# ApsaraDB/galaxysql

Hardware: NVIDIA H100
Metric: joined+aggregated rows/sec; achieved HBM GB/s vs peak, at 1/2/4/8 H100 (higher is better)
Workload: dtype int64

## Files before the change

### galaxysql_b200/csrc/common.cuh

```cuda
#pragma once

#include <cuda_runtime.h>
#include <stdint.h>
#include <stdio.h>
#include <string.h>

#include <string>
#include <vector>

#include "../../include/gsql_gpu.h"

struct ProfEntry {
    std::string name;
    int64_t launches = 0;
    double ms = 0;
    std::vector<std::pair<cudaEvent_t, cudaEvent_t>> pending;
};

struct gsql_ctx {
    int device = 0;
    cudaStream_t stream = nullptr;
    bool own_stream = false;
    cudaStream_t copy_in = nullptr;
    cudaStream_t copy_out = nullptr;
// ... 174 lines not shown
    if (utype == GSQL_T_FP64) return gsql_hash_i64(gsql_double_bits(__longlong_as_double(k.i)));
    return gsql_hash_i64(k.i);
}
__device__ __forceinline__ int32_t gsql_row_hash(const KeySet &ks, int64_t r) {
    uint32_t h = 0;
#pragma unroll 1
    for (int c = 0; c < ks.n; c++) {
        KeyVal k = gsql_load_key(ks.c[c], r, ks.utype[c]);
        h = h * 31u + (uint32_t)gsql_key_hash(k, ks.utype[c]);
    }
    return (int32_t)h;
}

__host__ __device__ __forceinline__ uint64_t gsql_fmix64(uint64_t x) {
    x ^= x >> 33;
    x *= 0xff51afd7ed558ccdULL;
    x ^= x >> 33;
    x *= 0xc4ceb9fe1a85ec53ULL;
    x ^= x >> 33;
    return x;
}

__device__ __forceinline__ int4 ld_stream_16(const void *p) { return __ldcs(reinterpret_cast<const int4 *>(p)); }
__device__ __forceinline__ long long ld_stream_8(const void *p) { return __ldcs(reinterpret_cast<const long long *>(p)); }
__device__ __forceinline__ int ld_stream_4(const void *p) { return __ldcs(reinterpret_cast<const int *>(p)); }
__device__ __forceinline__ void st_stream_16(void *p, const int4 &v) { __stcs(reinterpret_cast<int4 *>(p), v); }
__device__ __forceinline__ void st_stream_8(void *p, long long v) { __stcs(reinterpret_cast<long long *>(p), v); }
__device__ __forceinline__ void st_stream_4(void *p, int v) { __stcs(reinterpret_cast<int *>(p), v); }

__device__ __forceinline__ uint64_t l2_policy_evict_last() {
    uint64_t pol;
    asm volatile("createpolicy.fractional.L2::evict_last.b64 %0, 1.0;" : "=l"(pol));
    return pol;
}
__device__ __forceinline__ int4 ld_keep_16(const void *p, uint64_t pol) {
    int4 v;
    asm volatile("ld.global.nc.L2::cache_hint.v4.s32 {%0,%1,%2,%3}, [%4], %5;"
                 : "=r"(v.x), "=r"(v.y), "=r"(v.z), "=r"(v.w)
                 : "l"(p), "l"(pol));
    return v;
}
__device__ __forceinline__ int4 ld_keep_16_na(const void *p, uint64_t pol) {
    int4 v;
    asm volatile("ld.global.nc.L1::no_allocate.L2::cache_hint.v4.s32 {%0,%1,%2,%3}, [%4], %5;"
                 : "=r"(v.x), "=r"(v.y), "=r"(v.z), "=r"(v.w)
                 : "l"(p), "l"(pol));
    return v;
}
__device__ __forceinline__ unsigned long long ld_keep_8(const void *p, uint64_t pol) {
    unsigned long long v;
    asm volatile("ld.global.nc.L2::cache_hint.u64 %0, [%1], %2;" : "=l"(v) : "l"(p), "l"(pol));
    return v;
}

__device__ __forceinline__ void red_add_f64_keep(double *p, double v, uint64_t pol) {
    asm volatile("red.global.add.L2::cache_hint.f64 [%0], %1, %2;" ::"l"(p), "d"(v), "l"(pol) : "memory");
}
__device__ __forceinline__ void red_add_u64_keep(unsigned long long *p, unsigned long long v, uint64_t pol) {
    asm volatile("red.global.add.L2::cache_hint.u64 [%0], %1, %2;" ::"l"(p), "l"(v), "l"(pol) : "memory");
}
__device__ __forceinline__ unsigned int ld_keep_u8(const uint8_t *p, uint64_t pol) {
    unsigned int v;
    asm volatile("ld.global.L2::cache_hint.u8 %0, [%1], %2;" : "=r"(v) : "l"(p), "l"(pol));
    return v;
}

static inline int64_t div_up(int64_t a, int64_t b) { return (a + b - 1) / b; }

gsql_status local_split_by_slot_range(gsql_ctx *ctx, const DColSet &in, int key_col, int64_t rows, int nparts, void *const *out_data);
```

### galaxysql_b200/csrc/join.cu

```cuda
#include <cub/device/device_scan.cuh>
#include <cub/iterator/transform_input_iterator.cuh>

#include <stdlib.h>

#include "common.cuh"
#include "join_fast.cuh"

namespace {

constexpr unsigned long long DIGEST_EMPTY = 0x8000000000000000ULL;
enum { F_ANY_MULTI = 0, F_MORE_THAN_ONE = 1, F_NULL_INTO_NONNULL = 2, F_COUNT = 4 };
enum { SIDE_PROBE = 0, SIDE_BUILD = 1 };

struct __align__(16) Slot {
    unsigned long long digest;
    int head;
    int multi;
};

struct OutCol {
    void *data;
    uint8_t *nulls;
    int32_t type;
    int32_t side;
// ... 562 lines not shown
    int64_t nh = (int64_t)P * g.nblocks;
    DevBuf hist, offs, tmp;
    GSQL_TRY(hist.alloc(ctx, (size_t)(nh + 1) * 8));
    GSQL_TRY(offs.alloc(ctx, (size_t)(nh + 1) * 8));
    GSQL_CUDA(ctx, cudaMemsetAsync((char *)hist.p + nh * 8, 0, 8, ctx->stream));
    std::string name = std::string("join_fast_hist_") + tag;
    {
        KernelScope ks(ctx, name.c_str());
        if (rpt) {
            FJ_DISPATCH_MODE(direct, {
                fj::k_fj_hist<fj::SM_THREADS, DM><<<g.nblocks, fj::SM_THREADS, (size_t)P * 4, ctx->stream>>>(cols.c[L.key_col], g, hist.as<int64_t>(), flags, M);
            });
        } else {
            fj::k_fj_hist<fj::THREADS, false><<<g.nblocks, fj::THREADS, (size_t)P * 4, ctx->stream>>>(cols.c[L.key_col], g, hist.as<int64_t>(), flags, M);
        }
    }
    GSQL_CUDA(ctx, cudaGetLastError());
    size_t tb = 0;
    GSQL_CUDA(ctx, cub::DeviceScan::ExclusiveSum(nullptr, tb, hist.as<int64_t>(), offs.as<int64_t>(), nh + 1, ctx->stream));
    GSQL_TRY(tmp.alloc(ctx, tb));
    name = std::string("join_fast_scan_") + tag;
    {
        KernelScope ks(ctx, name.c_str());
        GSQL_CUDA(ctx, cub::DeviceScan::ExclusiveSum(tmp.p, tb, hist.as<int64_t>(), offs.as<int64_t>(), nh + 1, ctx->stream));
    }
    const bool pipe = fj_scatter_pipe(W, P);
    size_t smem = rpt ? fj::scatter_sm_smem_bytes(W, P, rpt) : fj::scatter_smem_bytes(W, P, pipe);
    name = std::string("join_fast_scatter_") + tag;
    {
        KernelScope ks(ctx, name.c_str());
        FJ_DISPATCH_W(W, {
            if (rpt) {
                FJ_DISPATCH_MODE(direct, {
                    GSQL_CUDA(ctx, cudaFuncSetAttribute(fj::k_fj_scatter_sm<WW, DM>, cudaFuncAttributeMaxDynamicSharedMemorySize, (int)smem));
                    fj::k_fj_scatter_sm<WW, DM><<<g.nblocks, fj::SM_THREADS, smem, ctx->stream>>>(cols, L, g, rpt, offs.as<int64_t>(), RG, out, flags, M);
                });
            } else if (env_i64("GSQL_JOIN_SCATTER_DIRECT", 0)) {
                fj::k_fj_scatter_direct<WW><<<g.nblocks, fj::THREADS, (size_t)P * 12, ctx->stream>>>(cols, L, g, offs.as<int64_t>(), out);
            } else if (pipe) {
                    GSQL_CUDA(ctx, cudaFuncSetAttribute(fj::k_fj_scatter<WW, true>, cudaFuncAttributeMaxDynamicSharedMemorySize, (int)smem));
                fj::k_fj_scatter<WW, true><<<g.nblocks, fj::THREADS, smem, ctx->stream>>>(cols, L, g, offs.as<int64_t>(), out);
            } else {
                    GSQL_CUDA(ctx, cudaFuncSetAttribute(fj::k_fj_scatter<WW, false>, cudaFuncAttributeMaxDynamicSharedMemorySize, (int)smem));
                fj::k_fj_scatter<WW, false><<<g.nblocks, fj::THREADS, smem, ctx->stream>>>(cols, L, g, offs.as<int64_t>(), out);
            }
        });
    }
    GSQL_CUDA(ctx, cudaGetLastError());
    return GSQL_OK;
}

static gsql_status fj_build_blocks(gsql_ctx *ctx, JoinFast &F, const unsigned long long *packed, int64_t rows, uint64_t spp) {
    const int W = F.bl.nwords;
    int lgB = 1;
    while (((2ll << lgB) * W * 8) <= (128ll << 10)) lgB++;
    const int64_t forced = env_i64("GSQL_JOIN_BUILD_BLOCK_SLOTS", 0);
    if (forced > 0) {
        int optin = 0;
        GSQL_CUDA(ctx, cudaDeviceGetAttribute(&optin, cudaDevAttrMaxSharedMemoryPerBlockOptin, ctx->device));
        lgB = 1;
        while ((2ll << lgB) <= forced && ((2ll << lgB) * W * 8) <= optin) lgB++;
    }
    const int64_t nb = (int64_t)((F.nslots + (1ull << lgB) - 1) >> lgB);
    const int64_t def_cap = rows / 16 + 65536;
    DevBuf fill, def, ndef;
    GSQL_TRY(fill.alloc(ctx, (size_t)nb * 4));
    GSQL_TRY(def.alloc(ctx, (size_t)def_cap * W * 8));
    GSQL_TRY(ndef.alloc(ctx, 8));
    GSQL_CUDA(ctx, cudaMemsetAsync(fill.p, 0, fill.bytes, ctx->stream));
    GSQL_CUDA(ctx, cudaMemsetAsync(ndef.p, 0, 8, ctx->stream));
    unsigned long long *table = F.table.as<unsigned long long>();
    int32_t *flags = F.flags.as<int32_t>();
    FJ_DISPATCH_W(W, FJ_DISPATCH_MODE(F.direct, {
        {
            KernelScope ks(ctx, "join_fast_build_split");
            const size_t smem = fj::split_smem_bytes(WW);
            GSQL_CUDA(ctx, cudaFuncSetAttribute(fj::k_fj_build_split<WW, DM>, cudaFuncAttributeMaxDynamicSharedMemorySize, (int)smem));
            int per_sm = 0;
            GSQL_CUDA(ctx, cudaOccupancyMaxActiveBlocksPerMultiprocessor(&per_sm, fj::k_fj_build_split<WW, DM>, fj::BS_THREADS, smem));
            if (per_sm < 1) per_sm = 1;
            const int64_t tile = (int64_t)fj::BS_THREADS * fj::bs_rpt(WW);
            int64_t grid = (int64_t)ctx->sm_count * per_sm;
            const int64_t tiles = div_up(rows, tile);
            if (grid > tiles) grid = tiles;
            const int64_t chunk = div_up(div_up(rows, grid), tile) * tile;
            grid = div_up(rows, chunk);
            fj::k_fj_build_split<WW, DM><<<(unsigned)grid, fj::BS_THREADS, smem, ctx->stream>>>(packed, rows, chunk, F.P, spp, F.nslots, lgB, table,
                                                                                             fill.as<unsigned int>(), def.as<unsigned long long>(),
                                                                                             ndef.as<unsigned long long>(), def_cap, flags, F.km);
        }
        GSQL_CUDA(ctx, cudaGetLastError());
        {
            KernelScope ks(ctx, "join_fast_build_slab");
            const size_t smem = ((size_t)1 << lgB) * WW * 8;
            GSQL_CUDA(ctx, cudaFuncSetAttribute(fj::k_fj_build_slab<WW, DM>, cudaFuncAttributeMaxDynamicSharedMemorySize, (int)smem));
            fj::k_fj_build_slab<WW, DM><<<(unsigned)nb, fj::BS_THREADS, smem, ctx->stream>>>(table, F.nslots, lgB, fill.as<unsigned int>(),
                                                                                            def.as<unsigned long long>(), ndef.as<unsigned long long>(),
                                                                                            def_cap, flags, F.km);
        }
        GSQL_CUDA(ctx, cudaGetLastError());
        {
            KernelScope ks(ctx, "join_fast_build_deferred");
            const int64_t tiles = div_up(def_cap, fj::TILE);
            const int grid = (int)(tiles < (int64_t)ctx->sm_count * 2 ? tiles : (int64_t)ctx->sm_count * 2);
            DColSet none;
            memset(&none, 0, sizeof(none));
            fj::k_fj_insert<WW, DM><<<grid, fj::THREADS, 0, ctx->stream>>>(def.as<unsigned long long>(), none, F.bl, def_cap, table, F.nslots, flags,
                                                                           ndef.as<unsigned long long>(), F.km);
        }
    }));
    GSQL_CUDA(ctx, cudaGetLastError());
    return GSQL_OK;
}

static gsql_status fast_build(gsql_join *j) {
    gsql_ctx *ctx = j->ctx;
    const gsql_join_spec &s = j->spec;
    JoinFast &F = j->fast;
    F.enabled = false;
    if (env_i64("GSQL_JOIN_NO_FAST", 0)) return GSQL_OK;
    if (s.nkeys != 1 || s.build_outer || j->single_join || s.n_cond > 0) return GSQL_OK;
    if (s.key_type[0] != GSQL_T_INT32 && s.key_type[0] != GSQL_T_INT64) return GSQL_OK;
    if (j->build_types[j->bkey_cols[0]] == GSQL_T_FP64 || j->probe_types[j->pkey_cols[0]] == GSQL_T_FP64) return GSQL_OK;
    if (s.key_type[0] == GSQL_T_INT32 && (j->build_types[j->bkey_cols[0]] != GSQL_T_INT32 || j->probe_types[j->pkey_cols[0]] != GSQL_T_INT32))
        return GSQL_OK;
    if (j->pass_nothing || j->pass_through || j->build_rows == 0) return GSQL_OK;
    for (int i = 0; i < j->n_build; i++)
        if (j->bhas_nulls[i]) return GSQL_OK;
    if (!fj::make_layout(j->build_types, j->n_build, j->bkey_cols[0], &F.bl)) return GSQL_OK;
    if (!fj::make_layout(j->probe_types, j->n_probe, j->pkey_cols[0], &F.pl)) return GSQL_OK;
    F.eligible = true;
    F.part_bytes = env_i64("GSQL_JOIN_PART_BYTES", 16ll << 20);
    if (F.part_bytes < 4096) F.part_bytes = 4096;
    F.sub_batch = env_i64("GSQL_JOIN_SUB_BATCH", 1ll << 30);
    if (F.sub_batch < fj::TILE) F.sub_batch = fj::TILE;
    F.part_min_rows = env_i64("GSQL_JOIN_PART_MIN_ROWS", 1ll << 20);
    const int BW = F.bl.nwords;
    DColSet build;
    KeySet bkeys;
    fill_build_cols(j, &build, &bkeys);
    int64_t want = j->build_rows * env_i64("GSQL_JOIN_SLOTS_PER_ROW", 3);
    if (want < 1024) want = 1024;
    const bool l2_table = !getenv("GSQL_JOIN_PART_BYTES");
    const int64_t l2_bytes = env_i64("GSQL_JOIN_L2_TABLE_BYTES", 64ll << 20);
    int64_t P, spp;
    F.direct = false;
    if (!env_i64("GSQL_JOIN_TMA", 0) && !env_i64("GSQL_JOIN_PROBE_PIPE", 0)) {
        long long range[2] = {LLONG_MAX, LLONG_MIN};
        DevBuf d_range;
        GSQL_TRY(d_range.alloc(ctx, sizeof(range)));
        GSQL_CUDA(ctx, cudaMemcpyAsync(d_range.p, range, sizeof(range), cudaMemcpyHostToDevice, ctx->stream));
        {
            KernelScope ks(ctx, "join_key_range");
            fj::k_fj_key_range<<<grid_rows(ctx, j->build_rows, 256, 8), 256, 0, ctx->stream>>>(build.c[F.bl.key_col], j->build_rows,
                                                                                                  d_range.as<long long>());
        }
        GSQL_CUDA(ctx, cudaGetLastError());
        GSQL_CUDA(ctx, cudaMemcpyAsync(range, d_range.p, sizeof(range), cudaMemcpyDeviceToHost, ctx->stream));
        GSQL_CUDA(ctx, cudaStreamSynchronize(ctx->stream));
        const uint64_t span = (uint64_t)range[1] - (uint64_t)range[0];
        int bits = 10;
        while (bits < 63 && (span >> bits) != 0) bits++;
        if (bits < 63 && (1ll << bits) <= want && range[0] != LLONG_MIN) {
            const int64_t nslots = 1ll << bits;
            spp = 1;
            while (spp < nslots && spp * 2 * BW * 8 <= F.part_bytes) spp *= 2;
            while (nslots / spp > fj::MAX_P) spp *= 2;
            if (l2_table && nslots * BW * 8 <= l2_bytes) spp = nslots;
            P = nslots / spp;
            int rb = 0, rp = 0;
            GSQL_TRY(fj_scatter_rpt(ctx, BW, (int)P, &rb));
            GSQL_TRY(fj_scatter_rpt(ctx, F.pl.nwords, (int)P, &rp));
            if (rb && rp) {
                F.direct = true;
                F.km.kmin = (unsigned long long)range[0];
                F.km.bits = bits;
                F.km.lgP = 0;
                while ((1ll << F.km.lgP) < P) F.km.lgP++;
            }
        }
    }
    if (!F.direct) {
        P = div_up(want * BW * 8, F.part_bytes);
        if (l2_table && want * BW * 8 <= l2_bytes) P = 1;
        if (P > fj::MAX_P) P = fj::MAX_P;
        if (P < 1) P = 1;
        spp = div_up(want, P);
    }
    F.P = (int)P;
    F.nslots = (uint64_t)(spp * P);
    GSQL_TRY(F.table.alloc(ctx, (size_t)F.nslots * BW * 8));
    GSQL_TRY(F.flags.alloc(ctx, fj::FL_COUNT * 4));
    GSQL_TRY(F.cursor.alloc(ctx, 16));
    GSQL_CUDA(ctx, cudaMemsetAsync(F.flags.p, 0, fj::FL_COUNT * 4, ctx->stream));
    DevBuf packed;
    const bool blocks = F.P > 1 && env_i64("GSQL_JOIN_BUILD_FUSED", 1);
    if (!blocks) {
        KernelScope ks(ctx, "join_fast_table_init");
        int grid = grid_rows(ctx, (int64_t)F.nslots, 256, 8);
        FJ_DISPATCH_W(BW, { fj::k_fj_table_init<WW><<<grid, 256, 0, ctx->stream>>>(F.table.as<unsigned long long>(), F.nslots); });
    }
    const unsigned long long *src = nullptr;
    if (F.P > 1) {
        GSQL_TRY(packed.alloc(ctx, (size_t)j->build_rows * BW * 8));
        GSQL_TRY(fj_partition(ctx, build, F.bl, j->build_rows, F.P, fj::Regions{}, packed.as<unsigned long long>(), F.flags.as<int32_t>(), "build",
                              F.direct, F.km));
        src = packed.as<unsigned long long>();
    }
    if (blocks) {
        GSQL_TRY(fj_build_blocks(ctx, F, src, j->build_rows, (uint64_t)spp));
    } else {
        KernelScope ks(ctx, "join_fast_insert");
        int64_t itiles = div_up(j->build_rows, fj::TILE);
        int grid = (int)(itiles < (int64_t)ctx->sm_count * 2 ? itiles : (int64_t)ctx->sm_count * 2);
        FJ_DISPATCH_W(BW, FJ_DISPATCH_MODE(F.direct, {
            fj::k_fj_insert<WW, DM><<<grid, fj::THREADS, 0, ctx->stream>>>(src, build, F.bl, j->build_rows, F.table.as<unsigned long long>(), F.nslots,
                                                                           F.flags.as<int32_t>(), nullptr, F.km);
        }));
    }
    GSQL_CUDA(ctx, cudaGetLastError());
    int32_t hf[fj::FL_COUNT];
    GSQL_CUDA(ctx, cudaMemcpyAsync(hf, F.flags.p, sizeof(hf), cudaMemcpyDeviceToHost, ctx->stream));
    GSQL_CUDA(ctx, cudaStreamSynchronize(ctx->stream));
    if (hf[fj::FL_SENTINEL] || hf[fj::FL_DUP] || hf[fj::FL_DISP]) {
        F.table.release();
        return GSQL_OK;
    }
    GSQL_CUDA(ctx, cudaMemsetAsync(F.flags.p, 0, fj::FL_COUNT * 4, ctx->stream));
    F.enabled = true;
    return GSQL_OK;
}


static gsql_status ensure_generic(gsql_join *j) {
    if (j->generic_built) return GSQL_OK;
    gsql_ctx *ctx = j->ctx;
    const gsql_join_spec &s = j->spec;
    j->nslots = (uint64_t)(j->build_rows * 2 > 64 ? j->build_rows * 2 : 64);
    GSQL_TRY(j->slots.alloc(ctx, (size_t)(j->nslots + 1) * sizeof(Slot)));
    GSQL_TRY(j->links.alloc(ctx, (size_t)(j->build_rows > 0 ? j->build_rows : 1) * 4));
    if (s.build_outer) {
        GSQL_TRY(j->used.alloc(ctx, (size_t)(j->build_rows > 0 ? j->build_rows : 1)));
        GSQL_CUDA(ctx, cudaMemsetAsync(j->used.p, 0, j->used.bytes, ctx->stream));
    }
    {
        KernelScope ks(ctx, "join_slots_init");
        k_slots_init<<<grid_rows(ctx, (int64_t)j->nslots + 1, 256, 8), 256, 0, ctx->stream>>>(j->slots.as<Slot>(), j->nslots + 1);
    }
    if (j->build_rows > 0) {
        DColSet build;
        KeySet bkeys;
        fill_build_cols(j, &build, &bkeys);
        KernelScope ks(ctx, "join_build");
// ... 640 lines not shown
```

### galaxysql_b200/csrc/join_fast.cuh

```cuda
#pragma once

#include <cub/block/block_scan.cuh>
#include <cub/device/device_scan.cuh>

#include "common.cuh"

namespace fj {

constexpr unsigned long long KEY_EMPTY = 0x8000000000000000ULL;
constexpr int THREADS = 512;
constexpr int RPT = 4;
constexpr int TILE = THREADS * RPT;
constexpr int MAX_WORDS = 4;
constexpr int MAX_P = 1024;
constexpr int MAX_DISP = 4096;
enum { FL_SENTINEL = 0, FL_DUP = 1, FL_DISP = 2, FL_NULLOUT = 3, FL_SPILL = 4, FL_COUNT = 5 };

struct Layout {
    int32_t nwords, ncols, key_col, key_i32;
    int32_t word[GSQL_MAX_COLS];
    int32_t half[GSQL_MAX_COLS];
};

static bool make_layout(const int32_t *types, int ncols, int key_col, Layout *L) {
// ... 95 lines not shown
    for (int k = 0; k < RPT; k++)
#pragma unroll
        for (int i = 0; i < W; i++) w[k][i] = 0;
#pragma unroll 1
    for (int c = 0; c < L.ncols; c++) {
        const DCol &col = cols.c[c];
        const bool is32 = col.type == GSQL_T_INT32, iskey = c == L.key_col;
        const int wi = L.word[c];
        const int sh = L.half[c] == 1 ? 32 : 0;
        unsigned long long v[RPT];
#pragma unroll
        for (int k = 0; k < RPT; k++) {
            int64_t r = base + k * THREADS;
            v[k] = 0;
            if (r < limit) {
                if (is32) {
                    int x = ld_stream_4(reinterpret_cast<const int *>(col.data) + r);
                    v[k] = iskey ? (unsigned long long)(long long)x : (unsigned long long)(unsigned)x;
                } else {
                    v[k] = (unsigned long long)ld_stream_8(reinterpret_cast<const long long *>(col.data) + r);
                }
            }
        }
#pragma unroll
        for (int k = 0; k < RPT; k++) {
            unsigned long long vv = v[k] << sh;
#pragma unroll
            for (int i = 0; i < W; i++)
                if (i == wi) w[k][i] |= vv;
        }
    }
}

template <int W>
__device__ __forceinline__ void pack_tile(const DColSet &cols, const Layout &L, int64_t base, int64_t limit, unsigned long long (&w)[RPT][W]) {
    switch (L.ncols) {
    case 1: pack_tile_nc<W, 1>(cols, L, base, limit, w); break;
    case 2: pack_tile_nc<W, 2>(cols, L, base, limit, w); break;
    case 3: pack_tile_nc<W, 3>(cols, L, base, limit, w); break;
    case 4: pack_tile_nc<W, 4>(cols, L, base, limit, w); break;
    default: pack_tile_generic<W>(cols, L, base, limit, w); break;
    }
}

__device__ __forceinline__ unsigned long long load_key(const DCol &col, int64_t r) {
    if (col.type == GSQL_T_INT32) return (unsigned long long)(long long)ld_stream_4(reinterpret_cast<const int *>(col.data) + r);
    return (unsigned long long)ld_stream_8(reinterpret_cast<const long long *>(col.data) + r);
}

__device__ __forceinline__ unsigned int part_of(uint64_t h, int P) { return __umulhi((unsigned int)(h >> 32), (unsigned int)P); }

struct KeyMap {
    unsigned long long kmin;
    int32_t bits, lgP;
};

template <bool DIRECT>
__device__ __forceinline__ uint64_t slot_of(unsigned long long k, uint64_t nslots, const KeyMap &M) {
    if (DIRECT) return ((k - M.kmin) * 0x9E3779B97F4A7C15ULL) & (nslots - 1);
    return __umul64hi(key_hash(k), nslots);
}

template <bool DIRECT>
__device__ __forceinline__ unsigned int part_of_key(unsigned long long k, int P, const KeyMap &M) {
    if (DIRECT) return (unsigned int)(slot_of<true>(k, 1ULL << M.bits, M) >> (M.bits - M.lgP));
    return part_of(key_hash(k), P);
}

__global__ void __launch_bounds__(256) k_fj_key_range(DCol keycol, int64_t n, long long *out) {
    constexpr int U = 4;
    long long lo = LLONG_MAX, hi = LLONG_MIN;
    const int64_t stride = (int64_t)gridDim.x * blockDim.x;
    for (int64_t r = (int64_t)blockIdx.x * blockDim.x + threadIdx.x; r < n; r += U * stride) {
        long long k[U];
#pragma unroll
        for (int u = 0; u < U; u++) k[u] = r + u * stride < n ? (long long)load_key(keycol, r + u * stride) : 0;
#pragma unroll
        for (int u = 0; u < U; u++) {
            if (r + u * stride >= n) continue;
            lo = k[u] < lo ? k[u] : lo;
            hi = k[u] > hi ? k[u] : hi;
        }
    }
#pragma unroll
    for (int d = 16; d > 0; d >>= 1) {
        const long long a = __shfl_xor_sync(0xffffffffu, lo, d), b = __shfl_xor_sync(0xffffffffu, hi, d);
        lo = a < lo ? a : lo;
        hi = b > hi ? b : hi;
    }
    if ((threadIdx.x & 31) == 0 && lo <= hi) {
        atomicMin(out, lo);
        atomicMax(out + 1, hi);
    }
}

struct PartGeom {
    int64_t rows, chunk;
    int32_t P, nblocks;
};

template <int NT, bool DIRECT>
__global__ void __launch_bounds__(NT) k_fj_hist(DCol keycol, PartGeom g, int64_t *__restrict__ hist, int32_t *flags, KeyMap M) {
    extern __shared__ unsigned int sh_hist[];
    for (int i = threadIdx.x; i < g.P; i += NT) sh_hist[i] = 0;
    __syncthreads();
    int64_t r0 = (int64_t)blockIdx.x * g.chunk;
    int64_t r1 = r0 + g.chunk < g.rows ? r0 + g.chunk : g.rows;
    bool sentinel = false;
    for (int64_t t0 = r0; t0 < r1; t0 += NT * RPT) {
        unsigned long long key[RPT];
#pragma unroll
        for (int k = 0; k < RPT; k++) {
            int64_t r = t0 + k * NT + threadIdx.x;
            key[k] = r < r1 ? load_key(keycol, r) : 0;
        }
#pragma unroll
        for (int k = 0; k < RPT; k++) {
            int64_t r = t0 + k * NT + threadIdx.x;
            if (r < r1) {
                sentinel |= key[k] == KEY_EMPTY;
                atomicAdd(&sh_hist[part_of_key<DIRECT>(key[k], g.P, M)], 1u);
            }
        }
    }
    if (sentinel) flags[FL_SENTINEL] = 1;
    __syncthreads();
    for (int i = threadIdx.x; i < g.P; i += NT) hist[(int64_t)i * g.nblocks + blockIdx.x] = sh_hist[i];
}

__device__ __forceinline__ void cp_async_4(void *smem_dst, const void *gsrc) {
    asm volatile("cp.async.ca.shared.global [%0], [%1], 4;" ::"r"((uint32_t)__cvta_generic_to_shared(smem_dst)), "l"(gsrc) : "memory");
}
__device__ __forceinline__ void cp_async_8(void *smem_dst, const void *gsrc) {
    asm volatile("cp.async.ca.shared.global [%0], [%1], 8;" ::"r"((uint32_t)__cvta_generic_to_shared(smem_dst)), "l"(gsrc) : "memory");
}
__device__ __forceinline__ void cp_async_16(void *smem_dst, const void *gsrc) {
    asm volatile("cp.async.cg.shared.global [%0], [%1], 16;" ::"r"((uint32_t)__cvta_generic_to_shared(smem_dst)), "l"(gsrc) : "memory");
}
__device__ __forceinline__ void cp_async_16_hint(void *smem_dst, const void *gsrc, uint64_t pol) {
    asm volatile("cp.async.cg.shared.global.L2::cache_hint [%0], [%1], 16, %2;" ::"r"((uint32_t)__cvta_generic_to_shared(smem_dst)), "l"(gsrc), "l"(pol)
                 : "memory");
}
__device__ __forceinline__ void cp_async_commit() { asm volatile("cp.async.commit_group;" ::: "memory"); }
template <int N>
__device__ __forceinline__ void cp_async_wait() { asm volatile("cp.async.wait_group %0;" ::"n"(N) : "memory"); }

__device__ __forceinline__ uint32_t smem_u32(const void *p) { return (uint32_t)__cvta_generic_to_shared(p); }
__device__ __forceinline__ void mbar_init(unsigned long long *bar, int count) {
    asm volatile("mbarrier.init.shared::cta.b64 [%0], %1;" ::"r"(smem_u32(bar)), "r"(count) : "memory");
}
__device__ __forceinline__ void mbar_expect_tx(unsigned long long *bar, uint32_t bytes) {
    asm volatile("mbarrier.arrive.expect_tx.shared::cta.b64 _, [%0], %1;" ::"r"(smem_u32(bar)), "r"(bytes) : "memory");
}
__device__ __forceinline__ void mbar_wait(unsigned long long *bar, uint32_t parity) {
    uint32_t done = 0;
    while (!done)
        asm volatile("{\n\t.reg .pred p;\n\tmbarrier.try_wait.parity.shared::cta.b64 p, [%1], %2;\n\tselp.u32 %0, 1, 0, p;\n\t}"
                     : "=r"(done) : "r"(smem_u32(bar)), "r"(parity) : "memory");
}
__device__ __forceinline__ uint64_t l2_policy_evict_first() {
    uint64_t pol;
    asm volatile("createpolicy.fractional.L2::evict_first.b64 %0, 1.0;" : "=l"(pol));
    return pol;
}
__device__ __forceinline__ void tma_load_1d(void *smem_dst, const void *gsrc, uint32_t bytes, unsigned long long *bar, uint64_t pol) {
    asm volatile("cp.async.bulk.shared::cluster.global.mbarrier::complete_tx::bytes.L2::cache_hint [%0], [%1], %2, [%3], %4;" ::"r"(smem_u32(smem_dst)),
                 "l"(gsrc), "r"(bytes), "r"(smem_u32(bar)), "l"(pol)
                 : "memory");
}

template <bool FULL>
__device__ __forceinline__ void tile_prefetch(const DColSet &cols, const Layout &L, int64_t t0, int n_tile, unsigned char *buf) {
    const unsigned tid = threadIdx.x;
    unsigned char *sp = buf + tid * 4u;
#pragma unroll 1
    for (int c = 0; c < L.ncols; c++) {
        const DCol &col = cols.c[c];
        if (col.type == GSQL_T_INT32) {
// ... 456 lines not shown
                } else {
#pragma unroll
                    for (int j = 0; j < W; j++) st_stream_8(out + dst * W + j, (long long)stage[(size_t)i * W + j]);
                }
            }
        }
    }
    if (K) {
        __syncthreads();
        if (tid < g.P) delta2[tid] = nxt;
        __syncthreads();
        for (int p = warp; p < g.P; p += SM_THREADS / 32) {
            const unsigned long long c = cur[p], e = (c | (K - 1)) + 1;
            const unsigned long long base = (unsigned long long)p * RG.cap, n0 = delta2[p];
            const unsigned long long n1 = n0 + K < (unsigned long long)RG.cap ? n0 + K : (unsigned long long)RG.cap;
            for (unsigned long long r = c + lane; r < e; r += 32) st_stream_8(out + r * W, (long long)KEY_EMPTY);
            for (unsigned long long r = base + n0 + lane; r < base + n1; r += 32) st_stream_8(out + r * W, (long long)KEY_EMPTY);
        }
    }
}

__global__ void __launch_bounds__(256) k_fj_region_tail(Regions RG, int W, unsigned long long *out) {
    const unsigned long long p = blockIdx.x, cap = (unsigned long long)RG.cap, f = RG.fill[p];
    for (unsigned long long r = p * cap + (f < cap ? f : cap) + threadIdx.x; r < (p + 1) * cap; r += 256)
        st_stream_8(out + r * W, (long long)KEY_EMPTY);
}

template <int W>
__global__ void __launch_bounds__(THREADS) k_fj_table_init(unsigned long long *table, uint64_t nslots) {
    for (uint64_t i = blockIdx.x * (uint64_t)blockDim.x + threadIdx.x; i < nslots; i += (uint64_t)gridDim.x * blockDim.x) {
        table[i * W] = KEY_EMPTY;
#pragma unroll
        for (int j = 1; j < W; j++) table[i * W + j] = 0;
    }
}

template <int W, bool DIRECT>
__global__ void __launch_bounds__(THREADS, 2) k_fj_insert(const unsigned long long *__restrict__ packed, const __grid_constant__ DColSet cols,
                                                       const __grid_constant__ Layout L, int64_t n, unsigned long long *table, uint64_t nslots,
                                                       int32_t *flags, const unsigned long long *n_dev, KeyMap M) {
    if (n_dev && *n_dev < (unsigned long long)n) n = (int64_t)*n_dev;
    for (int64_t t0 = (int64_t)blockIdx.x * TILE; t0 < n; t0 += (int64_t)gridDim.x * TILE) {
        unsigned long long w[RPT][W];
        if (packed) {
#pragma unroll
            for (int k = 0; k < RPT; k++) {
                int64_t r = t0 + k * THREADS + threadIdx.x;
#pragma unroll
                for (int i = 0; i < W; i++) w[k][i] = r < n ? (unsigned long long)ld_stream_8(packed + r * W + i) : 0;
            }
        } else {
            pack_tile<W>(cols, L, t0 + threadIdx.x, n, w);
        }
        uint64_t sl[RPT];
        unsigned long long prev[RPT];
        bool pending[RPT];
        bool any = false;
#pragma unroll
        for (int k = 0; k < RPT; k++) {
            int64_t r = t0 + k * THREADS + threadIdx.x;
            sl[k] = slot_of<DIRECT>(w[k][0], nslots, M);
            pending[k] = r < n;
            if (pending[k] && w[k][0] == KEY_EMPTY) { flags[FL_SENTINEL] = 1; pending[k] = false; }
            any |= pending[k];
        }
        int disp = 0;
        while (__any_sync(0xffffffffu, any)) {
#pragma unroll
            for (int k = 0; k < RPT; k++)
                if (pending[k]) prev[k] = atomicCAS(table + sl[k] * W, KEY_EMPTY, w[k][0]);
            any = false;
#pragma unroll
            for (int k = 0; k < RPT; k++) {
                if (!pending[k]) continue;
                if (prev[k] == KEY_EMPTY) {
#pragma unroll
                    for (int i = 1; i < W; i++) table[sl[k] * W + i] = w[k][i];
                    pending[k] = false;
                } else if (prev[k] == w[k][0]) {
                    flags[FL_DUP] = 1;
                    pending[k] = false;
                } else {
                    if (++sl[k] == nslots) sl[k] = 0;
                }
                any |= pending[k];
            }
            if (++disp > MAX_DISP) { if (any) flags[FL_DISP] = 1; break; }
        }
    }
}

constexpr int BS_THREADS = 512;
constexpr int BS_WIN = 2048;
__host__ __device__ constexpr int bs_rpt(int W) { return 12 / W; }

template <int W>
__device__ __forceinline__ void load_row(const unsigned long long *p, unsigned long long (&w)[W]) {
    if (W == 2) {
        const int4 v = ld_stream_16(p);
        w[0] = ((unsigned long long)(unsigned)v.y << 32) | (unsigned)v.x;
        w[W - 1] = ((unsigned long long)(unsigned)v.w << 32) | (unsigned)v.z;
    } else {
#pragma unroll
        for (int i = 0; i < W; i++) w[i] = (unsigned long long)ld_stream_8(p + i);
    }
}
// ... 46 lines not shown
        unsigned long long w[R][W];
        unsigned int br[R], n_staged;
#pragma unroll
        for (int k = 0; k < R; k++)
            if (k * BS_THREADS + tid < n_tile) load_row<W>(packed + (t0 + k * BS_THREADS + tid) * W, w[k]);
#pragma unroll
        for (int k = 0; k < R; k++) {
            br[k] = 0xffffffffu;
            if (k * BS_THREADS + tid >= n_tile) continue;
            const uint64_t rel = (slot_of<DIRECT>(w[k][0], nslots, M) >> lgB) - blo;
            if (rel < nwin) {
                br[k] = ((unsigned)rel << 16) | atomicAdd(&cnt[rel], 1u);
            } else {
                defer_row<W>(w[k], def, ndef, def_cap, flags);
            }
        }
        __syncthreads();
        {
            unsigned int v[IPT];
#pragma unroll
            for (int i = 0; i < IPT; i++) v[i] = cnt[tid * IPT + i];
            unsigned int c[IPT];
#pragma unroll
            for (int i = 0; i < IPT; i++) c[i] = v[i];
            BlockScan(scan_tmp).ExclusiveSum(v, v, n_staged);
#pragma unroll
            for (int i = 0; i < IPT; i++) {
                const unsigned e = tid * IPT + i;
                start[e] = v[i];
                if (c[i]) {
                    base[e] = atomicAdd(&fill[blo + e], c[i]);
                    cnt[e] = 0;
                }
            }
        }
        __syncthreads();
#pragma unroll
        for (int k = 0; k < R; k++) {
            if (br[k] == 0xffffffffu) continue;
            const unsigned pos = start[br[k] >> 16] + (br[k] & 0xffffu);
#pragma unroll
            for (int i = 0; i < W; i++) stage[(size_t)pos * W + i] = w[k][i];
            sb[pos] = (unsigned short)(br[k] >> 16);
        }
        __syncthreads();
        for (int i = tid; i < (int)n_staged; i += BS_THREADS) {
            const unsigned e = sb[i];
            const uint64_t s0 = (blo + e) << lgB;
            const uint64_t cap = nslots - s0 < (1ull << lgB) ? nslots - s0 : (1ull << lgB);
            const uint64_t pos = (uint64_t)base[e] + (unsigned)i - start[e];
            unsigned long long rw[W];
#pragma unroll
            for (int j = 0; j < W; j++) rw[j] = stage[(size_t)i * W + j];
            if (pos >= cap) { defer_row<W>(rw, def, ndef, def_cap, flags); continue; }
            unsigned long long *dst = table + (s0 + pos) * W;
            if (W == 2) {
                int4 v;
                v.x = (int)(unsigned)rw[0]; v.y = (int)(unsigned)(rw[0] >> 32);
                v.z = (int)(unsigned)rw[W - 1]; v.w = (int)(unsigned)(rw[W - 1] >> 32);
                *reinterpret_cast<int4 *>(dst) = v;
            } else {
#pragma unroll
                for (int j = 0; j < W; j++) dst[j] = rw[j];
            }
        }
    }
}

template <int W, bool DIRECT>
__global__ void __launch_bounds__(BS_THREADS) k_fj_build_slab(unsigned long long *table, uint64_t nslots, int lgB, const unsigned int *__restrict__ fill,
                                                              unsigned long long *def, unsigned long long *ndef, int64_t def_cap, int32_t *flags,
                                                              KeyMap M) {
    constexpr int R = bs_rpt(W) < 8 ? bs_rpt(W) : 8;
    extern __shared__ __align__(16) unsigned long long st[];
    const int tid = threadIdx.x;
    const uint64_t s0 = (uint64_t)blockIdx.x << lgB;
    const unsigned cap = (unsigned)(nslots - s0 < (1ull << lgB) ? nslots - s0 : (1ull << lgB));
    const unsigned n = fill[blockIdx.x] < cap ? fill[blockIdx.x] : cap;
    unsigned long long *g = table + s0 * W;
    for (unsigned i = tid; i < cap; i += BS_THREADS) {
        st[(size_t)i * W] = KEY_EMPTY;
#pragma unroll
        for (int j = 1; j < W; j++) st[(size_t)i * W + j] = 0;
    }
    __syncthreads();
    for (unsigned i0 = 0; i0 < n; i0 += BS_THREADS * R) {
        unsigned long long w[R][W];
#pragma unroll
        for (int k = 0; k < R; k++) {
            const unsigned i = i0 + k * BS_THREADS + tid;
            if (i < n) load_row<W>(g + (size_t)i * W, w[k]);
        }
#pragma unroll
        for (int k = 0; k < R; k++) {
            if (i0 + k * BS_THREADS + tid >= n) continue;
            const unsigned long long key = w[k][0];
            if (key == KEY_EMPTY) { flags[FL_SENTINEL] = 1; continue; }
            unsigned s = (unsigned)(slot_of<DIRECT>(key, nslots, M) - s0);
            int disp = 0;
            while (true) {
                if (s >= cap) { defer_row<W>(w[k], def, ndef, def_cap, flags); break; }
                const unsigned long long prev = atomicCAS(&st[(size_t)s * W], KEY_EMPTY, key);
                if (prev == KEY_EMPTY) {
#pragma unroll
                    for (int i = 1; i < W; i++) st[(size_t)s * W + i] = w[k][i];
                    break;
                }
                if (prev == key) { flags[FL_DUP] = 1; break; }
                ++s;
                if (++disp > MAX_DISP) { flags[FL_DISP] = 1; break; }
            }
        }
    }
    __syncthreads();
    const unsigned nw = cap * W;
    const int4 *s4 = reinterpret_cast<const int4 *>(st);
    for (unsigned i = tid; i < nw / 2; i += BS_THREADS) st_stream_16(g + (size_t)i * 2, s4[i]);
    if ((nw & 1) && tid == 0) st_stream_8(g + nw - 1, (long long)st[nw - 1]);
}

struct OutMap {
    void *data[GSQL_MAX_COLS * 2];
    uint8_t *nulls[GSQL_MAX_COLS * 2];
    int8_t side[GSQL_MAX_COLS * 2];
    int8_t word[GSQL_MAX_COLS * 2];
    int8_t half[GSQL_MAX_COLS * 2];
    int8_t is32[GSQL_MAX_COLS * 2];
    int32_t nout;
    int32_t join_type;
    int32_t stage_off[GSQL_MAX_COLS * 2];
    int32_t stage_null_off[GSQL_MAX_COLS * 2];
// ... 99 lines not shown
}
static size_t probe_pipe_smem_bytes(int PW, int BW) { return ((stage_words_bytes_c(PW, BW, 2048) + 15) & ~(size_t)15) + (size_t)2048 * PW * 8; }
static size_t stage_words_bytes(int PW, int BW, int tile_rows) {
    int BP = BW > 1 ? BW - 1 : 1;
    return (size_t)(PW + BP) * tile_rows * 8 + (size_t)tile_rows;
}

template <int R, int PW, int BP, int J>
__device__ __forceinline__ void write_col_h(int h, char *data, uint8_t *nulls, bool nu, const unsigned long long (&pw)[R][PW],
                                            const unsigned long long (&bp)[R][BP], const bool (&found)[R], const bool (&em)[R],
                                            const unsigned long long (&pos)[R], int32_t *flags) {
    if (h == 0) write_col<R, PW, BP, J, 0>(data, nulls, nu, pw, bp, found, em, pos, flags);
    else if (h == 1) write_col<R, PW, BP, J, 1>(data, nulls, nu, pw, bp, found, em, pos, flags);
    else write_col<R, PW, BP, J, 2>(data, nulls, nu, pw, bp, found, em, pos, flags);
}

template <int R, int PW, int BP>
__device__ __forceinline__ void write_rows(const OutMap &O, const unsigned long long (&pw)[R][PW], const unsigned long long (&bp)[R][BP],
                                           const bool (&found)[R], const bool (&em)[R], const unsigned long long (&pos)[R], int32_t *flags) {
#pragma unroll 1
    for (int q = 0; q < O.nout; q++) {
        const bool probe_side = O.side[q] == 0;
        const int j = probe_side ? O.word[q] : (O.word[q] == 0 ? 0 : PW + O.word[q] - 1);
        const int h = O.is32[q] ? (O.half[q] == 1 ? 1 : 0) : 2;
        char *data = reinterpret_cast<char *>(O.data[q]);
        uint8_t *nulls = O.nulls[q];
        const bool nu = !probe_side;
        switch (j) {
        case 0: write_col_h<R, PW, BP, 0>(h, data, nulls, nu, pw, bp, found, em, pos, flags); break;
        case 1: write_col_h<R, PW, BP, 1>(h, data, nulls, nu, pw, bp, found, em, pos, flags); break;
        case 2: write_col_h<R, PW, BP, 2>(h, data, nulls, nu, pw, bp, found, em, pos, flags); break;
        case 3: write_col_h<R, PW, BP, 3>(h, data, nulls, nu, pw, bp, found, em, pos, flags); break;
        case 4: write_col_h<R, PW, BP, 4>(h, data, nulls, nu, pw, bp, found, em, pos, flags); break;
        case 5: write_col_h<R, PW, BP, 5>(h, data, nulls, nu, pw, bp, found, em, pos, flags); break;
        default: write_col_h<R, PW, BP, 6>(h, data, nulls, nu, pw, bp, found, em, pos, flags); break;
        }
    }
}


template <int R, int PW, int BW, int BP, bool DIRECT = false>
__device__ __forceinline__ void lookup_rounds(const unsigned long long *__restrict__ table, uint64_t nslots, uint64_t pol,
                                              const unsigned long long (&pw)[R][PW], unsigned long long (&bp)[R][BP], bool (&found)[R],
                                              int mode = 0, int4 *gbuf = nullptr, const KeyMap &M = KeyMap{}) {
    uint64_t slot[R];
    unsigned long long tk[R];
    bool pending[R];
#pragma unroll
    for (int k = 0; k < R; k++) {
        slot[k] = slot_of<DIRECT>(pw[k][0], nslots, M);
#pragma unroll
        for (int i = 0; i < BP; i++) bp[k][i] = 0;
    }
    if (BW == 2 && mode == 2) {
#pragma unroll
        for (int k = 0; k < R; k++) cp_async_16_hint(gbuf + k * THREADS + threadIdx.x, table + slot[k] * 2, pol);
        cp_async_commit();
        cp_async_wait<0>();
#pragma unroll
        for (int k = 0; k < R; k++) {
            int4 v = gbuf[k * THREADS + threadIdx.x];
            tk[k] = ((unsigned long long)(unsigned)v.y << 32) | (unsigned)v.x;
            bp[k][0] = ((unsigned long long)(unsigned)v.w << 32) | (unsigned)v.z;
        }
    } else {
#pragma unroll
        for (int k = 0; k < R; k++) {
            if (BW == 2) {
                int4 v = mode == 1 ? ld_keep_16_na(table + slot[k] * 2, pol) : ld_keep_16(table + slot[k] * 2, pol);
                tk[k] = ((unsigned long long)(unsigned)v.y << 32) | (unsigned)v.x;
                bp[k][0] = ((unsigned long long)(unsigned)v.w << 32) | (unsigned)v.z;
            } else {
                tk[k] = ld_keep_8(table + slot[k] * BW, pol);
            }
        }
    }
    bool any = false;
#pragma unroll
    for (int k = 0; k < R; k++) {
        pending[k] = pw[k][0] != KEY_EMPTY && tk[k] != pw[k][0] && tk[k] != KEY_EMPTY;
        any |= pending[k];
    }
    while (!DIRECT && __any_sync(0xffffffffu, any)) {
#pragma unroll
        for (int k = 0; k < R; k++) {
            if (pending[k]) {
                if (++slot[k] == nslots) slot[k] = 0;
                if (BW == 2) {
                    int4 v = ld_keep_16(table + slot[k] * 2, pol);
                    tk[k] = ((unsigned long long)(unsigned)v.y << 32) | (unsigned)v.x;
                    bp[k][0] = ((unsigned long long)(unsigned)v.w << 32) | (unsigned)v.z;
                } else {
                    tk[k] = ld_keep_8(table + slot[k] * BW, pol);
                }
            }
        }
        any = false;
#pragma unroll
        for (int k = 0; k < R; k++) {
            pending[k] = pending[k] && tk[k] != pw[k][0] && tk[k] != KEY_EMPTY;
            any |= pending[k];
        }
    }
#pragma unroll
    for (int k = 0; k < R; k++) {
        found[k] = pw[k][0] != KEY_EMPTY && tk[k] == pw[k][0];
        if (BW > 2 && found[k]) {
#pragma unroll
            for (int i = 1; i < BW; i++) bp[k][i - 1] = ld_keep_8(table + slot[k] * BW + i, pol);
        }
    }
}

struct ProbeShared {
    unsigned int cell[THREADS / 32][RPT];
    unsigned long long tile_base;
    unsigned int tile_total;
};

template <int PW, int BW, bool DIRECT = false>
__device__ __forceinline__ void probe_tile(unsigned long long (&pw)[RPT][PW], const bool (&live)[RPT], const unsigned long long *__restrict__ table,
                                           uint64_t nslots, uint64_t pol, const OutMap &O, unsigned long long *cursor, int32_t *flags,
                                           ProbeShared &sh, unsigned char *probe_stage, const KeyMap &M = KeyMap{}) {
    constexpr int BP = BW > 1 ? BW - 1 : 1;
    const int lane = threadIdx.x & 31, warp = threadIdx.x >> 5;
    unsigned long long bp[RPT][BP];
    unsigned int ballot[RPT];
    bool found[RPT];
    lookup_rounds<RPT, PW, BW, BP, DIRECT>(table, nslots, pol, pw, bp, found, O.lookup_mode, reinterpret_cast<int4 *>(probe_stage), M);
#pragma unroll
    for (int k = 0; k < RPT; k++) {
        bool emit;
        switch (O.join_type) {
        case GSQL_JOIN_INNER: emit = found[k]; break;
        case GSQL_JOIN_SEMI: emit = found[k]; break;
        case GSQL_JOIN_ANTI: emit = !found[k]; break;
// ... 286 lines not shown
```

Baseline: 25.33 billion.

## Store direct-mapped join table as payload-only array plus occupancy bitmap

Measured after the change: 27.38 billion, median of 6. +8.1%, better.

```diff
diff --git a/galaxysql_b200/csrc/common.cuh b/galaxysql_b200/csrc/common.cuh
--- a/galaxysql_b200/csrc/common.cuh
+++ b/galaxysql_b200/csrc/common.cuh
@@ -250,6 +250,16 @@
     asm volatile("ld.global.nc.L2::cache_hint.u64 %0, [%1], %2;" : "=l"(v) : "l"(p), "l"(pol));
     return v;
 }
+__device__ __forceinline__ unsigned long long ld_keep_8_na(const void *p, uint64_t pol) {
+    unsigned long long v;
+    asm volatile("ld.global.nc.L1::no_allocate.L2::cache_hint.u64 %0, [%1], %2;" : "=l"(v) : "l"(p), "l"(pol));
+    return v;
+}
+__device__ __forceinline__ unsigned int ld_keep_4(const void *p, uint64_t pol) {
+    unsigned int v;
+    asm volatile("ld.global.nc.L2::cache_hint.u32 %0, [%1], %2;" : "=r"(v) : "l"(p), "l"(pol));
+    return v;
+}
 
 __device__ __forceinline__ void red_add_f64_keep(double *p, double v, uint64_t pol) {
     asm volatile("red.global.add.L2::cache_hint.f64 [%0], %1, %2;" ::"l"(p), "d"(v), "l"(pol) : "memory");
diff --git a/galaxysql_b200/csrc/join.cu b/galaxysql_b200/csrc/join.cu
--- a/galaxysql_b200/csrc/join.cu
+++ b/galaxysql_b200/csrc/join.cu
@@ -638,24 +638,32 @@
 
 static gsql_status fj_build_blocks(gsql_ctx *ctx, JoinFast &F, const unsigned long long *packed, int64_t rows, uint64_t spp) {
     const int W = F.bl.nwords;
-    int lgB = 1;
-    while (((2ll << lgB) * W * 8) <= (128ll << 10)) lgB++;
+    const int64_t slot_bits = F.direct ? (int64_t)(W - 1) * 64 + 1 : (int64_t)W * 64;
+    const int min_lgB = F.direct ? 5 : 1;
+    const int max_lgB = F.direct ? 16 : 62;
+    int lgB = min_lgB;
+    while (lgB < max_lgB && (2ll << lgB) * slot_bits / 8 <= (128ll << 10)) lgB++;
     const int64_t forced = env_i64("GSQL_JOIN_BUILD_BLOCK_SLOTS", 0);
     if (forced > 0) {
         int optin = 0;
         GSQL_CUDA(ctx, cudaDeviceGetAttribute(&optin, cudaDevAttrMaxSharedMemoryPerBlockOptin, ctx->device));
-        lgB = 1;
-        while ((2ll << lgB) <= forced && ((2ll << lgB) * W * 8) <= optin) lgB++;
+        lgB = min_lgB;
+        while (lgB < max_lgB && (2ll << lgB) <= forced && (2ll << lgB) * slot_bits / 8 <= optin) lgB++;
     }
     const int64_t nb = (int64_t)((F.nslots + (1ull << lgB) - 1) >> lgB);
     const int64_t def_cap = rows / 16 + 65536;
-    DevBuf fill, def, ndef;
+    DevBuf fill, def, ndef, scratch;
     GSQL_TRY(fill.alloc(ctx, (size_t)nb * 4));
     GSQL_TRY(def.alloc(ctx, (size_t)def_cap * W * 8));
     GSQL_TRY(ndef.alloc(ctx, 8));
     GSQL_CUDA(ctx, cudaMemsetAsync(fill.p, 0, fill.bytes, ctx->stream));
     GSQL_CUDA(ctx, cudaMemsetAsync(ndef.p, 0, 8, ctx->stream));
     unsigned long long *table = F.table.as<unsigned long long>();
+    unsigned long long *grouped = table;
+    if (F.direct) {
+        GSQL_TRY(scratch.alloc(ctx, (size_t)F.nslots * W * 8));
+        grouped = scratch.as<unsigned long long>();
+    }
     int32_t *flags = F.flags.as<int32_t>();
     FJ_DISPATCH_W(W, FJ_DISPATCH_MODE(F.direct, {
         {
@@ -671,16 +679,16 @@
             if (grid > tiles) grid = tiles;
             const int64_t chunk = div_up(div_up(rows, grid), tile) * tile;
             grid = div_up(rows, chunk);
-            fj::k_fj_build_split<WW, DM><<<(unsigned)grid, fj::BS_THREADS, smem, ctx->stream>>>(packed, rows, chunk, F.P, spp, F.nslots, lgB, table,
+            fj::k_fj_build_split<WW, DM><<<(unsigned)grid, fj::BS_THREADS, smem, ctx->stream>>>(packed, rows, chunk, F.P, spp, F.nslots, lgB, grouped,
                                                                                              fill.as<unsigned int>(), def.as<unsigned long long>(),
                                                                                              ndef.as<unsigned long long>(), def_cap, flags, F.km);
         }
         GSQL_CUDA(ctx, cudaGetLastError());
         {
             KernelScope ks(ctx, "join_fast_build_slab");
-            const size_t smem = ((size_t)1 << lgB) * WW * 8;
+            const size_t smem = (((size_t)1 << lgB) * slot_bits + 7) / 8;
             GSQL_CUDA(ctx, cudaFuncSetAttribute(fj::k_fj_build_slab<WW, DM>, cudaFuncAttributeMaxDynamicSharedMemorySize, (int)smem));
-            fj::k_fj_build_slab<WW, DM><<<(unsigned)nb, fj::BS_THREADS, smem, ctx->stream>>>(table, F.nslots, lgB, fill.as<unsigned int>(),
+            fj::k_fj_build_slab<WW, DM><<<(unsigned)nb, fj::BS_THREADS, smem, ctx->stream>>>(grouped, table, F.nslots, lgB, fill.as<unsigned int>(),
                                                                                             def.as<unsigned long long>(), ndef.as<unsigned long long>(),
                                                                                             def_cap, flags, F.km);
         }
@@ -747,7 +755,7 @@
         const uint64_t span = (uint64_t)range[1] - (uint64_t)range[0];
         int bits = 10;
         while (bits < 63 && (span >> bits) != 0) bits++;
-        if (bits < 63 && (1ll << bits) <= want && range[0] != LLONG_MIN) {
+        if (bits < 63 && (1ll << bits) <= want) {
             const int64_t nslots = 1ll << bits;
             spp = 1;
             while (spp < nslots && spp * 2 * BW * 8 <= F.part_bytes) spp *= 2;
@@ -760,6 +768,7 @@
             if (rb && rp) {
                 F.direct = true;
                 F.km.kmin = (unsigned long long)range[0];
+                F.km.dense = span + 1 == (uint64_t)j->build_rows ? span + 1 : 0;
                 F.km.bits = bits;
                 F.km.lgP = 0;
                 while ((1ll << F.km.lgP) < P) F.km.lgP++;
@@ -775,7 +784,7 @@
     }
     F.P = (int)P;
     F.nslots = (uint64_t)(spp * P);
-    GSQL_TRY(F.table.alloc(ctx, (size_t)F.nslots * BW * 8));
+    GSQL_TRY(F.table.alloc(ctx, F.direct ? fj::direct_table_bytes(BW, F.nslots) : (size_t)F.nslots * BW * 8));
     GSQL_TRY(F.flags.alloc(ctx, fj::FL_COUNT * 4));
     GSQL_TRY(F.cursor.alloc(ctx, 16));
     GSQL_CUDA(ctx, cudaMemsetAsync(F.flags.p, 0, fj::FL_COUNT * 4, ctx->stream));
@@ -783,8 +792,12 @@
     const bool blocks = F.P > 1 && env_i64("GSQL_JOIN_BUILD_FUSED", 1);
     if (!blocks) {
         KernelScope ks(ctx, "join_fast_table_init");
-        int grid = grid_rows(ctx, (int64_t)F.nslots, 256, 8);
-        FJ_DISPATCH_W(BW, { fj::k_fj_table_init<WW><<<grid, 256, 0, ctx->stream>>>(F.table.as<unsigned long long>(), F.nslots); });
+        if (F.direct) {
+            GSQL_CUDA(ctx, cudaMemsetAsync(F.table.as<unsigned long long>() + F.nslots * (BW - 1), 0, F.nslots / 8, ctx->stream));
+        } else {
+            int grid = grid_rows(ctx, (int64_t)F.nslots, 256, 8);
+            FJ_DISPATCH_W(BW, { fj::k_fj_table_init<WW><<<grid, 256, 0, ctx->stream>>>(F.table.as<unsigned long long>(), F.nslots); });
+        }
     }
     const unsigned long long *src = nullptr;
     if (F.P > 1) {
diff --git a/galaxysql_b200/csrc/join_fast.cuh b/galaxysql_b200/csrc/join_fast.cuh
--- a/galaxysql_b200/csrc/join_fast.cuh
+++ b/galaxysql_b200/csrc/join_fast.cuh
@@ -171,8 +171,20 @@
 
 struct KeyMap {
     unsigned long long kmin;
+    unsigned long long dense;
     int32_t bits, lgP;
 };
+
+__host__ __device__ constexpr size_t direct_table_bytes(int W, uint64_t nslots) { return (size_t)nslots * (W - 1) * 8 + nslots / 8; }
+
+template <int W>
+__device__ __forceinline__ unsigned int *direct_bitmap(unsigned long long *table, uint64_t nslots) {
+    return reinterpret_cast<unsigned int *>(table + nslots * (W - 1));
+}
+template <int W>
+__device__ __forceinline__ const unsigned int *direct_bitmap(const unsigned long long *table, uint64_t nslots) {
+    return reinterpret_cast<const unsigned int *>(table + nslots * (W - 1));
+}
 
 template <bool DIRECT>
 __device__ __forceinline__ uint64_t slot_of(unsigned long long k, uint64_t nslots, const KeyMap &M) {
@@ -242,7 +254,7 @@
             }
         }
     }
-    if (sentinel) flags[FL_SENTINEL] = 1;
+    if (!DIRECT && sentinel) flags[FL_SENTINEL] = 1;
     __syncthreads();
     for (int i = threadIdx.x; i < g.P; i += NT) hist[(int64_t)i * g.nblocks + blockIdx.x] = sh_hist[i];
 }
@@ -805,6 +817,22 @@
         } else {
             pack_tile<W>(cols, L, t0 + threadIdx.x, n, w);
         }
+        if constexpr (DIRECT) {
+            unsigned int *bm = direct_bitmap<W>(table, nslots);
+#pragma unroll
+            for (int k = 0; k < RPT; k++) {
+                if (t0 + k * THREADS + threadIdx.x >= n) continue;
+                const uint64_t s = slot_of<true>(w[k][0], nslots, M);
+                const unsigned int bit = 1u << (s & 31);
+                if (atomicOr(bm + (s >> 5), bit) & bit) {
+                    flags[FL_DUP] = 1;
+                    continue;
+                }
+#pragma unroll
+                for (int i = 1; i < W; i++) table[s * (W - 1) + i - 1] = w[k][i];
+            }
+            continue;
+        }
         uint64_t sl[RPT];
         unsigned long long prev[RPT];
         bool pending[RPT];
@@ -957,7 +985,11 @@
             unsigned long long rw[W];
 #pragma unroll
             for (int j = 0; j < W; j++) rw[j] = stage[(size_t)i * W + j];
-            if (pos >= cap) { defer_row<W>(rw, def, ndef, def_cap, flags); continue; }
+            if (pos >= cap) {
+                if (DIRECT) flags[FL_DUP] = 1;
+                else defer_row<W>(rw, def, ndef, def_cap, flags);
+                continue;
+            }
             unsigned long long *dst = table + (s0 + pos) * W;
             if (W == 2) {
                 int4 v;
@@ -973,15 +1005,52 @@
 }
 
 template <int W, bool DIRECT>
-__global__ void __launch_bounds__(BS_THREADS) k_fj_build_slab(unsigned long long *table, uint64_t nslots, int lgB, const unsigned int *__restrict__ fill,
-                                                              unsigned long long *def, unsigned long long *ndef, int64_t def_cap, int32_t *flags,
-                                                              KeyMap M) {
+__global__ void __launch_bounds__(BS_THREADS) k_fj_build_slab(const unsigned long long *grouped, unsigned long long *table, uint64_t nslots, int lgB,
+                                                              const unsigned int *__restrict__ fill, unsigned long long *def, unsigned long long *ndef,
+                                                              int64_t def_cap, int32_t *flags, KeyMap M) {
     constexpr int R = bs_rpt(W) < 8 ? bs_rpt(W) : 8;
     extern __shared__ __align__(16) unsigned long long st[];
     const int tid = threadIdx.x;
     const uint64_t s0 = (uint64_t)blockIdx.x << lgB;
     const unsigned cap = (unsigned)(nslots - s0 < (1ull << lgB) ? nslots - s0 : (1ull << lgB));
     const unsigned n = fill[blockIdx.x] < cap ? fill[blockIdx.x] : cap;
+    if constexpr (DIRECT) {
+        constexpr int BP = W - 1;
+        unsigned int *sbm = reinterpret_cast<unsigned int *>(st + (size_t)cap * BP);
+        for (unsigned i = tid; i < cap * BP; i += BS_THREADS) st[i] = 0;
+        for (unsigned i = tid; i < cap / 32; i += BS_THREADS) sbm[i] = 0;
+        __syncthreads();
+        const unsigned long long *g = grouped + s0 * W;
+        for (unsigned i0 = 0; i0 < n; i0 += BS_THREADS * R) {
+            unsigned long long w[R][W];
+#pragma unroll
+            for (int k = 0; k < R; k++) {
+                const unsigned i = i0 + k * BS_THREADS + tid;
+                if (i < n) load_row<W>(g + (size_t)i * W, w[k]);
+            }
+#pragma unroll
+            for (int k = 0; k < R; k++) {
+                if (i0 + k * BS_THREADS + tid >= n) continue;
+                const unsigned s = (unsigned)(slot_of<true>(w[k][0], nslots, M) - s0);
+                const unsigned int bit = 1u << (s & 31);
+                if (atomicOr(sbm + (s >> 5), bit) & bit) {
+                    flags[FL_DUP] = 1;
+                    continue;
+                }
+#pragma unroll
+                for (int i = 1; i < W; i++) st[(size_t)s * BP + i - 1] = w[k][i];
+            }
+        }
+        __syncthreads();
+        if (BP) {
+            unsigned long long *gp = table + s0 * BP;
+            const int4 *s4 = reinterpret_cast<const int4 *>(st);
+            for (unsigned i = tid; i < cap * BP / 2; i += BS_THREADS) st_stream_16(gp + (size_t)i * 2, s4[i]);
+        }
+        unsigned int *gbm = direct_bitmap<W>(table, nslots) + (s0 >> 5);
+        for (unsigned i = tid; i < cap / 32; i += BS_THREADS) st_stream_4(gbm + i, (int)sbm[i]);
+        return;
+    }
     unsigned long long *g = table + s0 * W;
     for (unsigned i = tid; i < cap; i += BS_THREADS) {
         st[(size_t)i * W] = KEY_EMPTY;
@@ -1187,6 +1256,25 @@
 #pragma unroll
         for (int i = 0; i < BP; i++) bp[k][i] = 0;
     }
+    if constexpr (DIRECT) {
+        const unsigned int *bm = direct_bitmap<BW>(table, nslots);
+        const unsigned long long lim = M.dense ? M.dense : nslots;
+        unsigned int bw[R];
+        bool in[R];
+#pragma unroll
+        for (int k = 0; k < R; k++) {
+            in[k] = pw[k][0] - M.kmin < lim;
+            bw[k] = 0xffffffffu;
+            if (in[k]) {
+                if (!M.dense) bw[k] = ld_keep_4(bm + (slot[k] >> 5), pol);
+#pragma unroll
+                for (int i = 0; i < BW - 1; i++) bp[k][i] = ld_keep_8_na(table + slot[k] * (BW - 1) + i, pol);
+            }
+        }
+#pragma unroll
+        for (int k = 0; k < R; k++) found[k] = in[k] && ((bw[k] >> (slot[k] & 31)) & 1u);
+        return;
+    }
     if (BW == 2 && mode == 2) {
 #pragma unroll
         for (int k = 0; k < R; k++) cp_async_16_hint(gbuf + k * THREADS + threadIdx.x, table + slot[k] * 2, pol);
@@ -1216,7 +1304,7 @@
         pending[k] = pw[k][0] != KEY_EMPTY && tk[k] != pw[k][0] && tk[k] != KEY_EMPTY;
         any |= pending[k];
     }
-    while (!DIRECT && __any_sync(0xffffffffu, any)) {
+    while (__any_sync(0xffffffffu, any)) {
 #pragma unroll
         for (int k = 0; k < R; k++) {
             if (pending[k]) {
```
